# MGI-tech-bioinformatics/SuperPlus

Hardware: AMD Instinct MI355X
Metric: k-mers/s (DF createDict stage: trim + canonical k-mer count + solid filter + spectrum + adjacency) (higher is better)
Workload: dtype u64

## Files before the change

### superplus_amd/csrc/dfk.hip

```cpp
#include "../../include/dfk.h"
#include "dfk_kernels.h"
#include "dfk_arena.h"

#include <algorithm>
#include <chrono>
#include <cstdarg>
#include <cstdio>
#include <cstdlib>
#include <cstring>
#include <atomic>
#include <fcntl.h>
#include <functional>
#include <new>
#include <string>
#include <sys/mman.h>
#include <sys/stat.h>
#include <unistd.h>
#include <condition_variable>
#include <memory>
#include <mutex>
#include <thread>
#include <vector>

using namespace dfk;
// ... 152 lines not shown
        budget += kept_budget; kept_budget = 0; kept_n_reads = 0;
    }
};

namespace {

struct Timer {
    hipEvent_t a{}, b{}; hipStream_t s;
    explicit Timer(hipStream_t st) : s(st) { (void)hipEventCreate(&a); (void)hipEventCreate(&b); }
    ~Timer() { (void)hipEventDestroy(a); (void)hipEventDestroy(b); }
    void start() { (void)hipEventRecord(a, s); }
    float stop() { (void)hipEventRecord(b, s); (void)hipEventSynchronize(b); float ms = 0; (void)hipEventElapsedTime(&ms, a, b); return ms; }
};

uint32_t ceil_log2(uint64_t v) { uint32_t b = 0; while ((1ull << b) < v) ++b; return b; }

template <int K>
int stage_trim(dfk_ctx* c, const Inputs& in, uint64_t* n_inst)
{
    DevBuf ctr; int rc = c->alloc(ctr, 32, "trim counters"); if (rc) return rc;
    HIP_TRY(hipMemsetAsync(ctr.p, 0, 32, c->stream));
    rc = c->alloc(c->good_len, sizeof(uint32_t) * in.n_reads, "goodLens", Place::Low); if (rc) return rc;
    if (in.n_reads) {
        unsigned grid = (unsigned)std::min<uint64_t>((in.n_reads + 255) / 256, 8192);
        hipLaunchKernelGGL(HIP_KERNEL_NAME(k_trim<K>), dim3(grid), dim3(256), 0, c->stream,
                           in.pq, in.pq_off, in.pq_bytes, in.base_off, in.packed_bytes, in.read_len, in.n_reads, c->cfg.min_qual, (uint32_t*)c->good_len.p,
                           (unsigned long long*)ctr.p, (unsigned int*)((char*)ctr.p + 8),
                           (unsigned long long*)((char*)ctr.p + 16));
        HIP_TRY(hipGetLastError());
    }
    uint64_t h[3] = {0, 0, 0};
    HIP_TRY(hipMemcpyAsync(h, ctr.p, 24, hipMemcpyDeviceToHost, c->stream));
    HIP_TRY(hipStreamSynchronize(c->stream));
    c->release(ctr);
    if ((uint32_t)h[1]) return fail(DFK_E_INPUT, "malformed input: an offset table is not monotone or runs past its array, a PQVec stream is broken, or its length differs from read_len");
    if (h[2] == 0) return fail(DFK_E_NOGOOD, "Looks like your input data have almost no good bases.");
    *n_inst = h[0];
    return 0;
}

int device_scan(dfk_ctx* c, const uint64_t* in, uint64_t* out, uint64_t n)
{
    constexpr uint64_t PER = (uint64_t)SCAN_THREADS * SCAN_ITEMS;
    if (n == 0) return 0;
    const uint64_t nblk = (n + PER - 1) / PER;
    if (nblk == 1) {
        hipLaunchKernelGGL(k_scan_blocks, dim3(1), dim3(SCAN_THREADS), 0, c->stream, in, out, n, (uint64_t*)nullptr);
// ... 125 lines not shown
    J->count_due = false;
    return 0;
}

template <int K>
int scan_keys_piece(dfk_ctx* c, const Inputs& in, BucketTable* T, ScanJob* J, uint64_t r0, uint64_t r1)
{
    static const unsigned scan_blocks = getenv("DFK_SCAN_BLOCKS") ? (unsigned)atoi(getenv("DFK_SCAN_BLOCKS")) : 0;
    const unsigned cus = (unsigned)c->prop.multiProcessorCount;
    const unsigned grid = (unsigned)std::min<uint64_t>((r1 - r0 + PART_THREADS - 1) / PART_THREADS, (uint64_t)(scan_blocks ? scan_blocks : 128u) * cus);
    const uint64_t n_subs = (uint64_t)J->n_cls * J->n_sub;
    const bool two = J->n_slices > 1;
    const uint32_t sl = two ? (uint32_t)(J->n_pieces & 1) : 0;
    hipStream_t ks = two ? c->stream2 : c->stream;
    auto* cnt = (unsigned long long*)J->sub.p;
    auto* off = cnt + n_subs;
    auto* cur = off + n_subs + 1;
    ScanKeys sk = J->sk;
    sk.keys = (uint32_t*)J->keys.p + (uint64_t)sl * sk.cap * J->n_cls;
    sk.fill = (unsigned long long*)J->fill.p + (uint64_t)sl * J->n_cls;
    if (two && J->n_pieces >= 2) HIP_TRY(hipStreamWaitEvent(c->stream, J->ev_part[sl], 0));
    HIP_TRY(hipMemsetAsync(sk.fill, 0, J->n_cls * 8, c->stream));
    const size_t lds = SCAN_RUN_LDS + SCAN_STAGE_LDS;
    hipLaunchKernelGGL(HIP_KERNEL_NAME(k_scan_count<K, 16, true>), dim3(grid), dim3(PART_THREADS), lds, c->stream,
                       in.packed, in.packed_bytes, in.base_off, (const uint32_t*)c->good_len.p, r0, r1, J->pp,
                       (unsigned long long*)T->acc.p, (unsigned long long*)nullptr, (unsigned long long*)J->d_n.p, J->ovf_cap,
                       (uint32_t*)J->ovf_tmp.p, (uint4*)T->summ.p, (uint32_t*)T->classes.p, sk);
    HIP_TRY(hipGetLastError());
    if (two) {
        HIP_TRY(hipEventRecord(J->ev_scan, c->stream));
        if (J->count_due) { int rc = scan_keys_count(c, T, J); if (rc) return rc; }
        HIP_TRY(hipStreamWaitEvent(ks, J->ev_scan, 0));
        if (J->n_pieces >= 1) HIP_TRY(hipStreamWaitEvent(ks, J->ev_count, 0));
    }
    HIP_TRY(hipMemsetAsync(cnt, 0, n_subs * 8, ks));
    const dim3 per_class(std::max(1u, 16u * cus / J->n_cls), J->n_cls);
    const uint32_t sh = 6 + J->sb;
    hipLaunchKernelGGL(k_keys_subcount, per_class, dim3(256), J->n_sub * 4, ks,
                       (const uint32_t*)sk.keys, (const unsigned long long*)sk.fill, sk.cap, sh, J->n_sub, cnt);
    HIP_TRY(hipGetLastError());
    hipLaunchKernelGGL(k_keys_offsets, dim3(1), dim3(1024), 0, ks, (const unsigned long long*)cnt, (uint32_t)n_subs, off, cur);
    HIP_TRY(hipGetLastError());
    hipLaunchKernelGGL(k_keys_partition, per_class, dim3(256), J->n_sub * 12, ks,
                       (const uint32_t*)sk.keys, (const unsigned long long*)sk.fill, sk.cap, sh, J->n_sub, cur, (uint32_t*)J->keys2.p);
    HIP_TRY(hipGetLastError());
    if (two) HIP_TRY(hipEventRecord(J->ev_part[sl], ks));
    ++J->n_pieces; J->count_due = true;
// ... 18 lines not shown
int scan_range(dfk_ctx* c, const Inputs& in, BucketTable* T, ScanJob* J, uint64_t r0, uint64_t r1)
{
    if (r1 <= r0) return 0;
    const PartParams& pp = J->pp;
    const bool by_class = J->by_class;
    unsigned grid = (unsigned)((r1 - r0 + PART_THREADS - 1) / PART_THREADS);
    static const unsigned scan_blocks = getenv("DFK_SCAN_BLOCKS") ? (unsigned)atoi(getenv("DFK_SCAN_BLOCKS")) : 0;
    if (by_class) grid = std::min<unsigned>(grid, (scan_blocks ? scan_blocks : 128u) * (unsigned)c->prop.multiProcessorCount);
    else if (scan_blocks) grid = std::min<unsigned>(grid, scan_blocks * (unsigned)c->prop.multiProcessorCount);
    const size_t lds_a = (sizeof(uint32_t) + 1) * pp.W * PART_THREADS + sizeof(uint32_t) * PART_RING * PART_THREADS + (by_class ? J->n_bins * 4 : 0);
    hipEvent_t e0, e1;
    HIP_TRY(hipEventCreate(&e0)); HIP_TRY(hipEventCreate(&e1));
    J->ev.emplace_back(e0, e1);
    HIP_TRY(hipEventRecord(e0, c->stream));
    if (J->keyed) {
        uint64_t p0 = r0;
        for (uint64_t m : scan_piece_sizes(J, r1 - r0, r1 == in.n_reads)) {
            int rc = scan_keys_piece<K>(c, in, T, J, p0, p0 + m); if (rc) return rc;
            p0 += m;
        }
        if (r1 == in.n_reads && J->count_due) { int rc = scan_keys_count(c, T, J); if (rc) return rc; }
    } else if (scan_takes_ranges<K>(c)) {
        const size_t lds_r = SCAN_RUN_LDS + (by_class ? J->n_bins * 4 : 0);
        hipLaunchKernelGGL(HIP_KERNEL_NAME(k_scan_count<K, 16, false>), dim3(grid), dim3(PART_THREADS), lds_r, c->stream,
                           in.packed, in.packed_bytes, in.base_off, (const uint32_t*)c->good_len.p, r0, r1, pp,
                           (unsigned long long*)T->acc.p, (unsigned long long*)T->class_hist.p, (unsigned long long*)J->d_n.p, J->ovf_cap,
                           (uint32_t*)J->ovf_tmp.p, (uint4*)T->summ.p, (uint32_t*)T->classes.p, ScanKeys{});
    } else {
        if (r0 != 0 || r1 != in.n_reads) return fail(DFK_E_STATE, "the general scan takes every read at once");
        hipLaunchKernelGGL(HIP_KERNEL_NAME(k_partition<K, false>), dim3(grid), dim3(PART_THREADS), lds_a, c->stream,
                           in.packed, in.packed_bytes, in.base_off, (const uint32_t*)c->good_len.p, in.bc,
                           (int64_t)c->cfg.ign_bc_below, in.n_reads, pp, (unsigned long long*)T->acc.p, (unsigned long long*)T->class_hist.p,
                           (unsigned long long*)J->d_n.p, J->ovf_cap, (uint4*)J->ovf_tmp.p, (uint4*)T->summ.p,
                           (const uint32_t*)nullptr, (uint64_t)0, (const uint64_t*)nullptr, (uint32_t*)T->classes.p);
    }
    HIP_TRY(hipGetLastError());
    HIP_TRY(hipEventRecord(e1, c->stream));
    return 0;
}

template <int K>
int scan_end(dfk_ctx* c, const Inputs& in, uint64_t n_inst, BucketTable* T, ScanJob* J)
{
    int rc = 0;
    T->n_ovf = 0;
    if (J->count_due) { rc = scan_keys_count(c, T, J); if (rc) return rc; }
    c->release(J->keys); c->release(J->keys2); c->release(J->fill); c->release(J->sub);
// ... 81 lines not shown
    c->release(rec); c->release(inst); c->release(flags); c->release(idx);
    return 0;
}

void release_pass(dfk_ctx* c, Partition* P)
{ c->release(P->records); c->release(P->base); c->release(P->ipre); c->release(P->items); }

template <int K> uint64_t item_budget(const dfk_ctx* c)
{
    constexpr uint64_t S = 1ull << CountCfg<K>::LOG2S;
    if (c->cfg.inst_per_item) return c->cfg.inst_per_item;
    if (c->distinct_per_inst <= 0.0) return 3 * S / 2;
    const double b = 0.367 * (double)S / c->distinct_per_inst;
    return (uint64_t)std::min(std::max(b, 0.5 * (double)S), 3.0 * (double)S);
}

struct ScatterJob { Partition P; DevBuf cur, d_bad; hipStream_t st = nullptr; hipEvent_t e0 = nullptr, e1 = nullptr; uint32_t lo = 0, n = 0; };

template <int K>
int scatter_launch(dfk_ctx* c, const Inputs& in, const BucketTable& T, uint32_t log2_world, int64_t read_id0, ScatterJob* J)
{
    const PartParams pp = part_params<K>(c, T.log2_nb, log2_world, read_id0, J->lo, J->n);
    HIP_TRY(hipEventRecord(J->e0, J->st));
    if (in.n_reads)
        hipLaunchKernelGGL(HIP_KERNEL_NAME(k_scatter_runs<K>), dim3((unsigned)((in.n_reads + 256ull * sweep_reads<K>() - 1) / (256ull * sweep_reads<K>()))),
                           dim3(256), 0, J->st,
                           in.packed, in.packed_bytes, in.base_off, (const uint32_t*)c->good_len.p, in.bc,
                           (int64_t)c->cfg.ign_bc_below, in.n_reads, pp, (const uint4*)T.summ.p, (const uint32_t*)T.classes.p,
                           (unsigned long long*)J->cur.p, J->P.n_records, (uint4*)J->P.records.p);
    HIP_TRY(hipGetLastError());
    HIP_TRY(hipEventRecord(J->e1, J->st));
    return 0;
}

template <int K>
int scatter_begin(dfk_ctx* c, const Inputs& in, const BucketTable& T, uint32_t log2_world, int64_t read_id0,
                  uint32_t sub_lo, uint32_t sub_n, ScatterJob* J, bool launch_now = true)
{
    Partition* P = &J->P;
    J->st = c->stream; J->lo = sub_lo; J->n = sub_n;
    const PartParams pp = part_params<K>(c, T.log2_nb, log2_world, read_id0, sub_lo, sub_n);
    const uint64_t budget = item_budget<K>(c);
    int rc = pass_tables(c, T.acc, T.log2_nb - log2_world, 1u << log2_world, sub_lo, sub_n, budget, P); if (rc) return rc;
    const uint64_t nb = P->nb;
    rc = c->alloc(J->cur, nb * 8, "bucket cursors"); if (rc) return rc;
    rc = c->alloc(P->records, P->n_records * 32, "super-k-mer records"); if (rc) return rc;
    rc = c->alloc(J->d_bad, 16, "scatter check"); if (rc) return rc;
    HIP_TRY(hipMemcpyAsync(J->cur.p, P->base.p, nb * 8, hipMemcpyDeviceToDevice, c->stream));
// ... 24 lines not shown
                               (unsigned long long*)J->cur.p, P->n_records, (uint4*)P->records.p, (uint4*)nullptr,
                               (const uint32_t*)T.ovf_list.p, T.n_ovf, (const uint64_t*)nullptr, (uint32_t*)nullptr);
        HIP_TRY(hipGetLastError());
        hipLaunchKernelGGL(k_check_cursors, dim3((unsigned)std::min<uint64_t>((P->nb + 255) / 256, 4096)), dim3(256), 0, c->stream, (const unsigned long long*)J->cur.p,
                           (const uint64_t*)P->base.p, P->nb, (unsigned int*)J->d_bad.p);
        HIP_TRY(hipGetLastError());
        c->st.ms_part_scatter += t.stop();
    }
    unsigned int bad = 0;
    HIP_TRY(hipMemcpy(&bad, J->d_bad.p, 4, hipMemcpyDeviceToHost));
    c->release(J->d_bad); c->release(J->cur);
    if (bad) return fail(DFK_E_HIP, "scatter: %u buckets did not receive the records counted for them (run summaries and bucket counters disagree)", bad);
    TRACE("scatter of buckets [%u, %u) done (%llu records, %llu items)", J->lo, J->lo + J->n,
          (unsigned long long)J->P.n_records, (unsigned long long)J->P.n_items);
    return 0;
}

constexpr int E_SPLIT_NO_ROOM = -101;
constexpr int E_SEGMENT_FULL = -100;

struct CountRun {
    CountGlobals* g = nullptr; uint4* seg = nullptr; unsigned long long* hist = nullptr;
    CountParams cp{}; unsigned grid = 0;
    DevBuf big; uint64_t big_cap = 0;
    DevBuf d_hist, d_g;
    DevBuf d_snap;
    DevBuf d_part;
    DevBuf d_wg;
    uint64_t solid_seen = 0, inst_seen = 0;
    uint64_t boundary_seen = 0;
    uint64_t splits_seen = 0;
};

int count_run_begin(dfk_ctx* c, CountRun* R)
{
    int rc = c->alloc(R->d_hist, (uint64_t)HIST_GLOBAL_BINS * 8, "spectrum bins", Place::Low); if (rc) return rc;
    rc = c->alloc(R->d_g, sizeof(CountGlobals), "count globals", Place::Low); if (rc) return rc;
    HIP_TRY(hipMemsetAsync(R->d_hist.p, 0, (uint64_t)HIST_GLOBAL_BINS * 8, c->stream));
    HIP_TRY(hipMemsetAsync(R->d_g.p, 0, sizeof(CountGlobals), c->stream));
    R->g = (CountGlobals*)R->d_g.p; R->hist = (unsigned long long*)R->d_hist.p;
    return c->alloc(R->d_snap, (uint64_t)HIST_GLOBAL_BINS * 8 + 256, "spectrum snapshot", Place::Low);
}

int count_snapshot(dfk_ctx* c, CountRun* R, bool restore)
{
    char* snap = (char*)R->d_snap.p;
// ... 27 lines not shown
#endif
    DevBuf d_max; int rc = c->alloc(d_max, 16, "max bin"); if (rc) return rc;
    HIP_TRY(hipMemsetAsync(d_max.p, 0, 16, c->stream));
    hipLaunchKernelGGL(k_hist_max, dim3(1024), dim3(256), 0, c->stream, (const unsigned long long*)R->d_hist.p, HIST_GLOBAL_BINS,
                       (unsigned int*)d_max.p);
    uint32_t nb = 0;
    HIP_TRY(hipMemcpyAsync(&nb, d_max.p, 4, hipMemcpyDeviceToHost, c->stream));
    HIP_TRY(hipStreamSynchronize(c->stream));
    c->hist.assign(nb, 0);
    if (nb) HIP_TRY(hipMemcpy(c->hist.data(), R->d_hist.p, 8ull * nb, hipMemcpyDeviceToHost));
    TRACE("spectrum read back: %u bins, %llu solid", nb, (unsigned long long)c->n_solid);
    c->release(d_max); c->release(R->d_hist); c->release(R->d_g); c->release(R->d_snap);
    return 0;
}

template <int K> unsigned count_grid(const dfk_ctx* c, int nbc = 1)
{
    constexpr int LOG2S = CountCfg<K>::LOG2S, NW = CountCfg<K>::NWAVES;
    const size_t lds = count_lds_bytes<K, LOG2S, NW, 1>() + (size_t)(nbc > 1 ? nbc - 1 : 0) * sizeof(uint32_t) * (1u << LOG2S);
    const unsigned per_cu = (unsigned)std::max<size_t>(1, (size_t)(160 * 1024) / lds);
    return (unsigned)c->prop.multiProcessorCount * per_cu;
}

int launch_boundary_list(dfk_ctx* c)
{
    if (c->pending_blist < 0) return 0;
    const dfk_ctx::Part& part = c->parts[(size_t)c->pending_blist];
    c->pending_blist = -1;
    unsigned long long* ctl = (unsigned long long*)((char*)part.buf.p + part.blist);
    HIP_TRY(hipMemsetAsync(ctl, 0, 16, c->stream2));
    hipLaunchKernelGGL(k_boundary_list, dim3((unsigned)std::min<uint64_t>((part.n + 2047) / 2048, 4096)), dim3(256), 0, c->stream2,
                       (const uint4*)part.buf.p, part.n, (uint32_t*)(ctl + 2), part.n_blist, ctl);
    HIP_TRY(hipGetLastError());
    return 0;
}

template <int K, int NBC>
int launch_count(dfk_ctx* c, const Partition& P, const ItemRange* d_items, uint64_t n_items, const CountRun& R,
                 std::vector<ItemRange>* overflowed, float* kernel_ms, const uint32_t* d_sub = nullptr, bool single_kmer_records = false)
{
    constexpr int LOG2S = CountCfg<K>::LOG2S, NW = CountCfg<K>::NWAVES;
    if (n_items == 0) return 0;
    if (n_items >= (1ull << 32)) return fail(DFK_E_ARG, "too many work items in one pass");
    DevBuf d_ovf;
    int rc = c->alloc(d_ovf, n_items * sizeof(ItemRange), "overflow list"); if (rc) return rc;
    HIP_TRY(hipMemsetAsync(&R.g->next_item, 0, 8, c->stream));
    HIP_TRY(hipMemsetAsync(&R.g->n_wg_idle, 0, 4, c->stream));
    CountParams cp = R.cp; cp.n_items = (uint32_t)n_items; cp.single = single_kmer_records ? 1u : 0u;
    const size_t lds = count_lds_bytes<K, LOG2S, NW, NBC>();
    auto kern = d_sub ? k_count<K, LOG2S, NW, NBC, true> : k_count<K, LOG2S, NW, NBC, false>;
    HIP_TRY(hipFuncSetAttribute(reinterpret_cast<const void*>(kern), hipFuncAttributeMaxDynamicSharedMemorySize, (int)lds));
    TRACE("k_count: %llu items, grid %u, lds %zu, seg_cap %llu", (unsigned long long)n_items, R.grid, lds, (unsigned long long)R.cp.seg_cap);
    Timer tk(c->stream);
    tk.start();
    hipLaunchKernelGGL(kern, dim3(R.grid), dim3(NW * 64), lds, c->stream,
                       (const uint4*)P.records.p, d_items, (const uint64_t*)P.base.p, cp, R.g, R.seg, (WgOut*)R.d_wg.p, R.hist,
                       (ItemRange*)d_ovf.p, d_sub, c->d_resident);
    HIP_TRY(hipGetLastError());
    c->resident_target += R.grid;
    if (c->after_count_launch || c->pending_blist >= 0) {
        hipLaunchKernelGGL(k_gate, dim3(1), dim3(64), 0, c->stream2, (const unsigned int*)c->d_resident, c->resident_target, 200000ull, c->d_resident + 1);
    }
    if (c->after_count_launch) { std::function<int()> f; f.swap(c->after_count_launch); rc = f(); if (rc) return rc; }
    rc = launch_boundary_list(c); if (rc) return rc;
    *kernel_ms += tk.stop();
    CountGlobals g{};
    HIP_TRY(hipMemcpyAsync(&g, R.g, sizeof g, hipMemcpyDeviceToHost, c->stream));
    HIP_TRY(hipStreamSynchronize(c->stream));
    c->last_wg_idle = g.n_wg_idle;
    if (g.n_overflow) {
        const size_t at = overflowed->size();
        overflowed->resize(at + g.n_overflow);
        HIP_TRY(hipMemcpy(overflowed->data() + at, d_ovf.p, sizeof(ItemRange) * g.n_overflow, hipMemcpyDeviceToHost));
    }
    c->release(d_ovf);
    return 0;
}

template <int K, int NBC>
int launch_count_big(dfk_ctx* c, const Partition& P, const std::vector<ItemRange>& singles, CountRun& R)
{
    constexpr int KW = KTraits<K>::KW, NW = 8;
    const uint32_t n = (uint32_t)singles.size();
    std::vector<uint32_t> idx(2 * n);
    for (uint32_t i = 0; i < n; ++i) { idx[2 * i] = singles[i].b0; idx[2 * i + 1] = singles[i].b1; }
    DevBuf d_idx, d_val;
    int rc = c->alloc(d_idx, 8ull * n, "gather index"); if (rc) return rc;
    rc = c->alloc(d_val, 16ull * n, "gather values"); if (rc) return rc;
    HIP_TRY(hipMemcpyAsync(d_idx.p, idx.data(), 8ull * n, hipMemcpyHostToDevice, c->stream));
    hipLaunchKernelGGL(k_gather_u64, dim3((2 * n + 255) / 256), dim3(256), 0, c->stream, (const uint64_t*)P.ipre.p,
                       (const uint32_t*)d_idx.p, 2 * n, (uint64_t*)d_val.p);
    HIP_TRY(hipGetLastError());
    std::vector<uint64_t> val(2 * n);
    HIP_TRY(hipMemcpyAsync(val.data(), d_val.p, 16ull * n, hipMemcpyDeviceToHost, c->stream));
    HIP_TRY(hipStreamSynchronize(c->stream));
    c->release(d_idx); c->release(d_val);
    std::vector<BigItem> items; uint64_t words = 0, tot_inst = 0;
    std::vector<uint64_t> chunk_pre(n + 1, 0), slot_pre(n + 1, 0), rec(2 * n);
    {
// ... 175 lines not shown
        DevBuf d_next; rc = c->alloc(d_next, next.size() * sizeof(ItemRange), "split items"); if (rc) return undo(rc);
        HIP_TRY(hipMemcpyAsync(d_next.p, next.data(), next.size() * sizeof(ItemRange), hipMemcpyHostToDevice, c->stream));
        rc = launch_count<K, NBC>(c, P2, (const ItemRange*)d_next.p, next.size(), R, &overflowed, &ignored, nullptr, true);
        if (rc) return undo(rc);
    }
    TRACE("fallback: %u buckets (%llu instances) split into %llu sub-buckets, %llu items; %zu sub-buckets to HBM tables", n, (unsigned long long)tot,
          (unsigned long long)ns, (unsigned long long)P2.n_items, singles.size());
    if (!singles.empty()) { rc = launch_count_big<K, NBC>(c, P2, singles, R); if (rc) return undo(rc); }
    HIP_TRY(hipStreamSynchronize(c->stream));
    c->release_since(mark, &R.big);
    return 0;
}

int barcode_words(const dfk_ctx* c, bool have_bc)
{ return !have_bc ? 0 : (int)std::max<uint32_t>(1, std::min<uint32_t>(c->cfg.min_bc, DFK_MAX_MIN_BC) - (c->cfg.min_bc > 1 ? 1 : 0)); }

template <int K> constexpr uint64_t out_chunk() { return 2ull << CountCfg<K>::LOG2S; }

template <int K>
int count_prepare(dfk_ctx* c, const Partition& P, CountRun& R, int nbc)
{
    const unsigned attempt = c->seg_attempt;
    R.grid = (unsigned)std::max<uint64_t>(1, std::min<uint64_t>(P.n_items, count_grid<K>(c, nbc)));
    uint64_t res = part_entries(P.n_inst, c->cfg.min_freq, R.inst_seen, R.solid_seen);
    res = (res << attempt) + (uint64_t)R.grid * out_chunk<K>();
    const uint64_t room = c->budget > c->held ? (c->budget - c->held) : 0;
    if (res * 32 > room) res = room / 32;
    int rc = c->alloc(R.d_wg, sizeof(WgOut) * R.grid, "workgroup output state"); if (rc) return rc;
    std::vector<WgOut> init(R.grid, WgOut{~0ull, (unsigned int)out_chunk<K>(), 0u});
    HIP_TRY(hipMemcpy(R.d_wg.p, init.data(), sizeof(WgOut) * R.grid, hipMemcpyHostToDevice));
    HIP_TRY(hipMemsetAsync(&R.g->big_cursor, 0, 8, c->stream));
    HIP_TRY(hipMemsetAsync(&R.g->part_cursor, 0, 8, c->stream));
    R.cp = CountParams{c->cfg.min_freq, c->cfg.min_bc, 0, 0, res, c->cfg.min_freq > 1 ? 1u : 0u,
                       (c->cfg.flags & DFK_F_KEEP_PRE_ADJ) ? 1u : 0u};
    R.big_cap = 0;
    rc = c->alloc(R.d_part, std::max<uint64_t>(1, res) * 32, "solid k-mer entries", Place::Low); if (rc) return rc;
    R.seg = (uint4*)R.d_part.p;
    return 0;
}

template <int K, int NBC>
int count_run(dfk_ctx* c, const Partition& P, CountRun& R)
{
    int rc = 0;
    Timer t(c->stream);
    std::vector<ItemRange> overflowed;
// ... 360 lines not shown
            if (r != DFK_E_NOMEM || forced || n <= 16 || ++retries > 12) return r;
            c->plan_derate *= 0.7;
            TRACE("out of HBM (%s): planning smaller passes", g_err.c_str());
        }
    };
    rc = start_alone(cur, 0); if (rc) return rc;
    while (cur.valid) {
        const uint32_t lo = cur.sj.lo, n = cur.sj.n, nlo = lo + n;
        rc = scatter_end<K>(c, in, T, 0, 0, &cur.sj); if (rc) return rc;
        const dfk_stats st0 = c->st;
        rc = count_snapshot(c, &R, false); if (rc) return rc;
        { Arena::Current in_blk(c->arena, cur.blk); rc = count_prepare<K>(c, cur.sj.P, R, barcode_words(c, in.bc != nullptr)); }
        nxt.valid = false;
        if (!rc && overlap && nlo < sub_nb) {
            const Partition& P = cur.sj.P;
            (void)P;
            const RunningPass rp{cur.blk.block.bytes, cur.sj.P.n_inst, n, c->arena.offset_of(cur.blk.block)};
            const uint32_t n2 = forced ? std::min(per_forced, sub_nb - nlo) : plan_range(plan_inputs(c, T, R, sub_nb, nlo, overlap), c->arena.free_blocks(), &rp);
            if (n2) {
                const int r2 = start(nxt, nlo, n2, true);
                if (r2 && r2 != DFK_E_NOMEM) return r2;
            }
        }
        if (!rc) {
            switch (barcode_words(c, in.bc != nullptr)) {
            case 0: rc = count_run<K, 0>(c, cur.sj.P, R); break;
            case 1: rc = count_run<K, 1>(c, cur.sj.P, R); break;
            case 2: rc = count_run<K, 2>(c, cur.sj.P, R); break;
            case 3: rc = count_run<K, 3>(c, cur.sj.P, R); break;
            case 4: rc = count_run<K, 4>(c, cur.sj.P, R); break;
            case 5: rc = count_run<K, 5>(c, cur.sj.P, R); break;
            case 6: rc = count_run<K, 6>(c, cur.sj.P, R); break;
            default: rc = count_run<K, 7>(c, cur.sj.P, R); break;
            }
        }
        if (c->after_count_launch) {
            std::function<int()> f; f.swap(c->after_count_launch);
            if (!rc) { const int r3 = f(); if (r3) return r3; } else nxt.valid = false;
        }
        if (rc == DFK_E_NOMEM || rc == E_SEGMENT_FULL) {
            HIP_TRY(hipStreamSynchronize(c->stream)); HIP_TRY(hipStreamSynchronize(c->stream2));
            c->release_since(cur.mark);
            R.d_wg = R.big = R.d_part = DevBuf{};
            drop_events(cur); drop_events(nxt); nxt.valid = false;
            int rc2 = count_snapshot(c, &R, true); if (rc2) return rc2;
            const float ms_scatter = c->st.ms_part_scatter, ms_count = c->st.ms_count, ms_fb = c->st.ms_fallback;
// ... 689 lines not shown
```

### superplus_amd/csrc/dfk_kernels.h

```cpp
#pragma once
#include <type_traits>
#include "dfk_device.h"

namespace dfk {

template <int K>
__global__ void __launch_bounds__(256)
k_trim(const uint8_t* __restrict__ pq, const uint64_t* __restrict__ pq_off, uint64_t pq_nbytes,
       const uint64_t* __restrict__ base_off, uint64_t packed_bytes, const uint32_t* __restrict__ read_len,
       uint64_t n_reads, uint32_t min_qual, uint32_t* __restrict__ good_len,
       unsigned long long* __restrict__ n_inst, unsigned int* __restrict__ bad,
       unsigned long long* __restrict__ sum_good)
{
    unsigned long long mine = 0, good = 0;
    bool any_bad = false;
    for (uint64_t r = (uint64_t)blockIdx.x * blockDim.x + threadIdx.x; r < n_reads; r += (uint64_t)gridDim.x * blockDim.x) {
        uint32_t gl = 0;
        uint64_t p = pq_off[r], end = pq_off[r + 1];
        uint32_t idx = 0, run = 0;
        const uint64_t b0 = base_off[r], b1 = base_off[r + 1];
        bool ok = p <= end && end <= pq_nbytes && b0 <= b1 && b1 <= packed_bytes && b1 - b0 >= ((uint64_t)read_len[r] + 3) / 4;
        if (!ok) end = p;
        while (p < end) {
            uint32_t nQs = pq[p];
            if (!nQs) break;
            if (p + 3 > end) { ok = false; break; }
            uint32_t hdr = pq[p + 1] | ((uint32_t)pq[p + 2] << 8);
            uint32_t nBits = hdr & 7u, minQ = (hdr >> 3) & 63u;
            uint64_t blk = ((uint64_t)nQs * nBits + 24) >> 3;
            if (p + blk > end) { ok = false; break; }
            if (nBits == 0) {
                if (minQ >= min_qual) { run += nQs; if (run >= (uint32_t)K) gl = idx + nQs; }
                else run = 0;
                idx += nQs;
            } else {
                uint64_t bit = 8 * (p + 1) + 9;
                const uint32_t fmask = (1u << nBits) - 1u;
                for (uint32_t left = nQs; left;) {
                    const uint64_t by = bit >> 3;
                    const uint32_t sh = (uint32_t)(bit & 7);
                    uint64_t w = 0;
                    if (by + 8 <= pq_nbytes) __builtin_memcpy(&w, pq + by, 8);
                    else for (uint32_t k = 0; k < 8 && by + k < pq_nbytes; ++k) w |= (uint64_t)pq[by + k] << (8 * k);
                    w >>= sh;
                    const uint32_t n = min(left, (64u - sh) / nBits);
                    for (uint32_t i = 0; i < n; ++i, w >>= nBits) {
                        const uint32_t q = minQ + ((uint32_t)w & fmask);
                        if (q < min_qual) run = 0;
                        else if (++run >= (uint32_t)K) gl = idx + 1;
                        ++idx;
                    }
                    bit += (uint64_t)n * nBits; left -= n;
                }
            }
            p += blk;
        }
        uint32_t rl = read_len[r];
        if (!ok || idx != rl) { any_bad = true; gl = 0; }
        if (gl > rl) gl = rl;
        good_len[r] = gl;
        good += gl;
        if (gl >= (uint32_t)K + 1) mine += gl - K + 1;
    }
    __shared__ unsigned long long sh[2][4];
    __shared__ unsigned int sh_bad;
    if (threadIdx.x == 0) sh_bad = 0;
    __syncthreads();
#pragma unroll
    for (int d = 32; d > 0; d >>= 1) { mine += __shfl_down(mine, d, 64); good += __shfl_down(good, d, 64); }
    if ((threadIdx.x & 63) == 0) { sh[0][threadIdx.x >> 6] = mine; sh[1][threadIdx.x >> 6] = good; }
    if (any_bad) atomicOr(&sh_bad, 1u);
    __syncthreads();
    if (threadIdx.x == 0) {
        unsigned long long a0 = sh[0][0] + sh[0][1] + sh[0][2] + sh[0][3], a1 = sh[1][0] + sh[1][1] + sh[1][2] + sh[1][3];
        if (a0) atomicAdd(n_inst, a0);
        if (a1) atomicAdd(sum_good, a1);
        if (sh_bad) atomicOr(bad, 1u);
    }
}

struct PartParams {
    uint32_t M;
    uint32_t W;
    uint32_t log2_nb;
    uint32_t log2_world;
// ... 6 lines not shown
constexpr uint32_t SWEEP_CLASSES = 32;
__host__ __device__ inline uint32_t sweep_class_of(uint32_t local_bucket, uint32_t log2_local)
{ return log2_local > 5 ? local_bucket >> (log2_local - 5) : local_bucket; }
__host__ __device__ inline uint32_t sweep_class_mask(uint32_t sub_lo, uint32_t sub_n, uint32_t log2_local)
{
    if (sub_n == 0) return 0u;
    const uint32_t a = sweep_class_of(sub_lo, log2_local), b = sweep_class_of(sub_lo + sub_n - 1, log2_local);
    const uint32_t upto_b = b >= 31 ? 0xFFFFFFFFu : ((1u << (b + 1)) - 1u);
    return upto_b & ~((1u << a) - 1u);
}

constexpr int PART_THREADS = 128;
constexpr int PART_RING = 2;
constexpr int SUMMARY_RUNS = 10;
constexpr uint32_t SUMMARY_OVERFLOW = 15;

__device__ __forceinline__ uint32_t pass_local(uint32_t bucket, const PartParams& pp)
{
    const uint32_t ls = pp.log2_nb - pp.log2_world;
    const uint32_t d = (bucket & ((1u << ls) - 1u)) - pp.sub_lo;
    return d < pp.sub_n ? (bucket >> ls) * pp.sub_n + d : 0xFFFFFFFFu;
}

__device__ __forceinline__ uint32_t bucket_of(uint32_t minhash, const PartParams& pp)
{
    const uint32_t b = (minhash * 0x9E3779B1u) >> (32 - pp.log2_nb);
    return ((b & ((1u << pp.log2_world) - 1u)) << (pp.log2_nb - pp.log2_world)) | (b >> pp.log2_world);
}
constexpr int PART_QCAP = 8;

template <int K>
__device__ __forceinline__ void emit_record(const uint32_t* __restrict__ words, uint64_t n_words, uint64_t bit0,
                                            uint32_t s0, uint32_t nk, uint32_t bucket, uint32_t gl, int32_t tag,
                                            uint64_t dst_index, uint4* __restrict__ records)
{
    const bool hp = s0 > 0;
    const bool hs = s0 + nk + (uint32_t)K <= gl;
    uint64_t bo = bit0 + 2ull * (hp ? s0 - 1 : 0);
    uint64_t wi = bo >> 5; uint32_t sh = (uint32_t)bo & 31u;
    uint32_t w[7];
#pragma unroll
    for (int i = 0; i < 7; ++i) w[i] = (wi + i < n_words) ? words[wi + i] : 0u;
    uint32_t o[6];
#pragma unroll
    for (int i = 0; i < 6; ++i) o[i] = alignbit(w[i + 1], w[i], sh);
    if (!hp) {
#pragma unroll
        for (int i = 5; i > 0; --i) o[i] = (o[i] << 2) | (o[i - 1] >> 30);
        o[0] <<= 2;
// ... 213 lines not shown
                                 bucket_acc, bucket_cur, n_out, records, summaries, read_list, n_list, slice_base, read_classes);
    if (lh) {
        __syncthreads();
        for (uint32_t i = threadIdx.x; i < n_bins; i += PART_THREADS) if (lh[i]) atomicAdd(&class_hist[i], (unsigned long long)lh[i]);
    }
}

template <int I, int N, class F>
__device__ __forceinline__ void static_for(F&& f)
{
    if constexpr (I < N) { f(std::integral_constant<int, I>{}); static_for<I + 1, N>(f); }
}

struct ScanKeys {
    uint32_t* keys;
    unsigned long long* fill;
    uint64_t cap;
    uint32_t ib;
};
constexpr int SCAN_STAGE = 1536;
constexpr uint32_t KEY_SUB_BITS = 14;
constexpr uint32_t KEY_TILE = 4096;

template <int K, int M, bool KEYS>
__global__ void __launch_bounds__(PART_THREADS)
k_scan_count(const uint8_t* __restrict__ packed, uint64_t packed_bytes, const uint64_t* __restrict__ base_off,
             const uint32_t* __restrict__ good_len, uint64_t r_first, uint64_t n_reads , PartParams pp,
             unsigned long long* __restrict__ bucket_acc, unsigned long long* __restrict__ class_hist,
             unsigned long long* __restrict__ ovf_count, uint64_t ovf_cap, uint32_t* __restrict__ ovf_list,
             uint4* __restrict__ summaries, uint32_t* __restrict__ read_classes, ScanKeys sk)
{
    constexpr int W = K - M + 1;
    constexpr uint32_t mmask = M == 16 ? 0xFFFFFFFFu : ((1u << (2 * M)) - 1u);
    constexpr uint32_t rsh = 2 * (M - 1);
    constexpr int RUNS = SUMMARY_RUNS;
    static_assert(KTraits<K>::NK_MAX < 64, "nk takes the key's six low bits");
    extern __shared__ uint32_t smem[];
    uint32_t* runb = smem;
    uint16_t* runf = reinterpret_cast<uint16_t*>(runb + RUNS * PART_THREADS);
    uint32_t* const after_runs = reinterpret_cast<uint32_t*>(runf + RUNS * PART_THREADS);
    uint32_t* lh = nullptr;
    const uint32_t n_bins = 2u * (PART_CLASSES << pp.log2_world);
    if (class_hist) {
        lh = after_runs;
        for (uint32_t i = threadIdx.x; i < n_bins; i += PART_THREADS) lh[i] = 0;
        __syncthreads();
    }
// ... 79 lines not shown
                uint32_t a[NA];
                {
                    const uint32_t sh = (uint32_t)nbit & 31u;
#pragma unroll
                    for (int i = 0; i < NA; ++i) a[i] = alignbit(i + 1 < NW ? nw[i + 1] : 0u, nw[i], sh);
                }
                nbit += 2 * W;
                load(nbit, nw);
                static_for<0, W>([&](auto bi_c) {
                    constexpr int bi = decltype(bi_c)::value;
                    if (t0 + (uint32_t)bi < n_mmers) {
                        const uint32_t b = (a[(2 * bi) >> 5] >> ((2 * bi) & 31)) & 3u;
                        f = ((f << 2) | b) & mmask;
                        rc = (rc >> 2) | ((3u - b) << rsh);
                        const uint32_t h = mmer_hash(f < rc ? f : rc);
                        const bool newmin = bi == 0 || h < P;
                        P = newmin ? h : P;
                        Pi = newmin ? (uint32_t)bi : Pi;
                        const bool first = t0 == 0;
                        if (!first || bi == W - 1) {
                            uint32_t mv = P;
                            bool older = false;
                            if constexpr (bi != W - 1) { older = arr[bi + 1] < mv; mv = older ? arr[bi + 1] : mv; }
                            const uint32_t bucket = bucket_of(mv, pp);
                            const bool open = first || bucket != cur_b || cur_nk == (uint32_t)KTraits<K>::NK_MAX;
                            if (open && !first) close_run();
                            const uint32_t rel = (bi != W - 1 && older) ? sidx_get(bi + 1 < W ? bi + 1 : 0) - (uint32_t)bi - 1u : (uint32_t)(W - 1 - bi) + Pi;
                            cur_rel = open ? rel : cur_rel;
                            cur_nk = open ? 1u : cur_nk + 1u;
                            cur_b = open ? bucket : cur_b;
                        }
                        arr[bi] = h;
                        if (bi == W - 1) {
                            uint32_t run = h, ri = W - 1;
                            sidx_set(W - 1, W - 1);
                            static_for<0, W - 1>([&](auto j_c) {
                                constexpr int i = W - 2 - decltype(j_c)::value;
                                const bool lt = arr[i] < run; run = lt ? arr[i] : run; arr[i] = run; ri = lt ? (uint32_t)i : ri; sidx_set(i, ri);
                            });
                        }
                    }
                });
            }
            close_run();
        }
        const uint32_t mine = min(qn, (uint32_t)RUNS);
        for (uint32_t i = 0; KEYS ? __syncthreads_or(i < mine) != 0 : __ballot(i < mine) != 0ull; ++i) {
// ... 146 lines not shown
        key_tile_each(t0, t1, v, [&](uint32_t key) { const uint32_t s = key >> sh2; out[base[s] + atomicAdd(&lh[s], 1u)] = key; });
        __syncthreads();
    }
}

__global__ void __launch_bounds__(1024)
k_keys_count(const uint32_t* __restrict__ part, const unsigned long long* __restrict__ off, uint32_t sb, unsigned long long* __restrict__ bucket_acc)
{
    __shared__ unsigned long long t[1u << KEY_SUB_BITS];
    const uint32_t s = blockIdx.x, nt = 1u << sb, m = nt - 1u;
    for (uint32_t i = threadIdx.x; i < nt; i += blockDim.x) t[i] = 0;
    __syncthreads();
    const uint64_t a = off[s], b = off[s + 1];
    for (uint64_t i = a + threadIdx.x; i < b; i += blockDim.x) {
        const uint32_t key = part[i];
        atomicAdd(&t[(key >> 6) & m], (1ull << 32) | (key & 63u));
    }
    __syncthreads();
    unsigned long long* dst = bucket_acc + ((uint64_t)s << sb);
    for (uint32_t i = threadIdx.x; i < nt; i += blockDim.x) if (t[i]) atomicAdd(&dst[i], t[i]);
}

constexpr int SLICE_READS = 16;
template <int K, bool EMIT, typename F>
__device__ __forceinline__ void for_each_run_in_pass(uint64_t r, const uint8_t* __restrict__ packed, uint64_t packed_bytes,
                                                     const uint64_t* __restrict__ base_off, const PartParams& pp,
                                                     const uint4* __restrict__ summaries, F&& f)
{
    const uint4 sm = summaries[r];
    const uint32_t n = sm.x & 15u;
    if (n == 0 || n == SUMMARY_OVERFLOW) return;
    const uint32_t* words = reinterpret_cast<const uint32_t*>(packed);
    const uint64_t n_words = (packed_bytes + 3) >> 2;
    const uint64_t bit0 = base_off[r] * 8;
    const uint32_t M = pp.M;
    const uint32_t mmask = M == 16 ? 0xFFFFFFFFu : ((1u << (2 * M)) - 1u);
    const uint64_t lo = (uint64_t)sm.x | ((uint64_t)sm.y << 32), hi = (uint64_t)sm.z | ((uint64_t)sm.w << 32);
    uint32_t s0 = 0;
#pragma unroll
    for (int i = 0; i < SUMMARY_RUNS; ++i) {
        if ((uint32_t)i < n) {
            constexpr int B0 = 8;
            const int b = B0 + 12 * i;
            const uint32_t fld = (uint32_t)(b + 12 <= 64 ? lo >> b : b >= 64 ? hi >> (b - 64) : (lo >> b) | (hi << (64 - b))) & 0xFFFu;
            const uint32_t nk = fld & 63u, rel = fld >> 6;
            const uint64_t bo = bit0 + 2ull * (s0 + rel);
            const uint64_t wi = bo >> 5;
            const uint32_t w0 = words[wi], w1 = wi + 1 < n_words ? words[wi + 1] : 0u;
            const uint32_t x = alignbit(w1, w0, (uint32_t)bo & 31u) & mmask;
            uint32_t y = __brev(x);
            y = ((y >> 1) & 0x55555555u) | ((y & 0x55555555u) << 1);
            const uint32_t fw = y >> (32 - 2 * M), rcv = ~x & mmask;
            const uint32_t bucket = bucket_of(mmer_hash(fw < rcv ? fw : rcv), pp);
            const uint32_t lb = pass_local(bucket, pp);
            if (lb != 0xFFFFFFFFu) f(s0, nk, lb, bucket >> (pp.log2_nb - pp.log2_world), bit0, (uint32_t)i + 1 == n);
            s0 += nk;
        }
    }
}

template <int K>
__global__ void __launch_bounds__(256)
k_scatter_slices(const uint8_t* __restrict__ packed, uint64_t packed_bytes, const uint64_t* __restrict__ base_off,
                 const uint32_t* __restrict__ good_len, const int32_t* __restrict__ bc, int64_t ign_bc_below,
                 uint64_t n_reads, PartParams pp, const uint4* __restrict__ summaries, const uint32_t* __restrict__ read_classes,
                 const uint64_t* __restrict__ slice_base,
                 unsigned long long* __restrict__ slice_fill,
                 uint4* __restrict__ records)
{
    __shared__ uint32_t cnt[256];
    __shared__ unsigned long long at[256];
    __shared__ uint16_t list[256 * SLICE_READS];
    __shared__ uint32_t n_list;
    const uint32_t world = 1u << pp.log2_world;
    const int lane = threadIdx.x & 63;
    const uint64_t r_block = (uint64_t)blockIdx.x * 256 * SLICE_READS;
// ... 22 lines not shown
        at[threadIdx.x] = slice_base[threadIdx.x] + (m ? atomicAdd(&slice_fill[threadIdx.x], (unsigned long long)m) : 0ull);
        cnt[threadIdx.x] = 0;
    }
    __syncthreads();
    const uint32_t* words = reinterpret_cast<const uint32_t*>(packed);
    const uint64_t n_words = (packed_bytes + 3) >> 2;
    (void)good_len;
    for (uint32_t i = threadIdx.x; i < n; i += 256) {
        const uint64_t r = r_block + list[i];
        int32_t tag = -1;
        if (bc && (int64_t)r + pp.read_id0 >= ign_bc_below) tag = bc[r];
        for_each_run_in_pass<K, true>(r, packed, packed_bytes, base_off, pp, summaries,
            [&](uint32_t s0, uint32_t nk, uint32_t lb, uint32_t owner, uint64_t bit0, bool last) {
                const uint64_t dst = at[owner] + atomicAdd(&cnt[owner], 1u);
                if (dst < slice_base[owner + 1]) emit_record<K>(words, n_words, bit0, s0, nk, lb, last ? 0u : 0xFFFFFFFFu, tag, dst, records);
            });
    }
}

#ifndef DFK_SWEEP_READS
#define DFK_SWEEP_READS 8
#endif
template <int K> constexpr int sweep_reads() { return KTraits<K>::KW == 4 ? 2 : DFK_SWEEP_READS; }
template <int K>
__global__ void __launch_bounds__(256)
k_scatter_runs(const uint8_t* __restrict__ packed, uint64_t packed_bytes, const uint64_t* __restrict__ base_off,
               const uint32_t* __restrict__ good_len, const int32_t* __restrict__ bc, int64_t ign_bc_below,
               uint64_t n_reads, PartParams pp, const uint4* __restrict__ summaries, const uint32_t* __restrict__ read_classes,
               unsigned long long* __restrict__ bucket_cur, uint64_t n_out, uint4* __restrict__ records)
{
    constexpr int SWEEP_READS = sweep_reads<K>();
    __shared__ uint16_t list[256 * SWEEP_READS];
    __shared__ uint32_t n_list;
    (void)good_len;
    const int lane = threadIdx.x & 63;
    const uint64_t r_block = (uint64_t)blockIdx.x * 256 * SWEEP_READS;
    if (threadIdx.x == 0) n_list = 0;
    __syncthreads();
#pragma unroll
    for (int j = 0; j < SWEEP_READS; ++j) {
        const uint32_t rel = 256u * j + threadIdx.x;
        const uint64_t r = r_block + rel;
        const bool hit = r < n_reads && (read_classes[r] & pp.class_mask) != 0u;
        const unsigned long long mk = __ballot(hit);
        uint32_t at = 0;
        if (lane == 0 && mk) at = atomicAdd(&n_list, (uint32_t)__popcll(mk));
        at = __builtin_amdgcn_readfirstlane(at);
        if (hit) list[at + __popcll(mk & ((1ull << lane) - 1ull))] = (uint16_t)rel;
    }
    __syncthreads();
    const uint32_t n = n_list;
    const uint32_t* words = reinterpret_cast<const uint32_t*>(packed);
    const uint64_t n_words = (packed_bytes + 3) >> 2;
    for (uint32_t i = threadIdx.x; i < n; i += 256) {
        const uint64_t r = r_block + list[i];
        int32_t tag = -1;
        if (bc && (int64_t)r + pp.read_id0 >= ign_bc_below) tag = bc[r];
        for_each_run_in_pass<K, true>(r, packed, packed_bytes, base_off, pp, summaries,
            [&](uint32_t s0, uint32_t nk, uint32_t lb, uint32_t, uint64_t bit0, bool last) {
                const uint64_t dst = atomicAdd(&bucket_cur[lb], 1ull);
                if (dst < n_out) emit_record<K>(words, n_words, bit0, s0, nk, lb, last ? 0u : 0xFFFFFFFFu, tag, dst, records);
            });
    }
}



struct ItemRange { uint32_t b0, b1; };

struct CountParams {
    uint32_t min_freq, min_bc;
    uint32_t n_items;
    uint32_t single;
    uint64_t seg_cap;
    uint32_t do_adj;
    uint32_t keep_pre;
};

struct CountGlobals {
    unsigned long long n_distinct;
    unsigned long long big_cursor;
// ... 1466 lines not shown
```

Before: 64.75 billion.

## Batch trim reads per thread, specialize single-device bucketing, add wider count shape

The trim kernel now has each thread prefetch offsets and the first quality header for two reads before walking them. It also handles a leading constant-quality block without the byte loop, and the grid is sized from occupancy. Scan and scatter kernels gain a SOLO template path that skips the world-interleave arithmetic in bucket_of when log2_world is zero. The count kernel can also launch with 12 waves per block when the LDS fits two blocks per CU and there is at most one barcode word, which raises parallelism per block at the cost of more template instantiations.

```diff
diff --git a/superplus_amd/csrc/dfk.hip b/superplus_amd/csrc/dfk.hip
--- a/superplus_amd/csrc/dfk.hip
+++ b/superplus_amd/csrc/dfk.hip
@@ -198,7 +198,10 @@
     HIP_TRY(hipMemsetAsync(ctr.p, 0, 32, c->stream));
     rc = c->alloc(c->good_len, sizeof(uint32_t) * in.n_reads, "goodLens", Place::Low); if (rc) return rc;
     if (in.n_reads) {
-        unsigned grid = (unsigned)std::min<uint64_t>((in.n_reads + 255) / 256, 8192);
+        const uint64_t per_block = 256ull * TRIM_READS;
+        int per_cu = 0;
+        HIP_TRY(hipOccupancyMaxActiveBlocksPerMultiprocessor(&per_cu, reinterpret_cast<const void*>(&k_trim<K>), 256, 0));
+        unsigned grid = (unsigned)std::min<uint64_t>((in.n_reads + per_block - 1) / per_block, (uint64_t)std::max(1, per_cu) * (uint64_t)c->prop.multiProcessorCount);
         hipLaunchKernelGGL(HIP_KERNEL_NAME(k_trim<K>), dim3(grid), dim3(256), 0, c->stream,
                            in.pq, in.pq_off, in.pq_bytes, in.base_off, in.packed_bytes, in.read_len, in.n_reads, c->cfg.min_qual, (uint32_t*)c->good_len.p,
                            (unsigned long long*)ctr.p, (unsigned int*)((char*)ctr.p + 8),
@@ -370,7 +373,8 @@
     if (two && J->n_pieces >= 2) HIP_TRY(hipStreamWaitEvent(c->stream, J->ev_part[sl], 0));
     HIP_TRY(hipMemsetAsync(sk.fill, 0, J->n_cls * 8, c->stream));
     const size_t lds = SCAN_RUN_LDS + SCAN_STAGE_LDS;
-    hipLaunchKernelGGL(HIP_KERNEL_NAME(k_scan_count<K, 16, true>), dim3(grid), dim3(PART_THREADS), lds, c->stream,
+    auto kern = J->pp.log2_world == 0 ? k_scan_count<K, 16, true, true> : k_scan_count<K, 16, true, false>;
+    hipLaunchKernelGGL(kern, dim3(grid), dim3(PART_THREADS), lds, c->stream,
                        in.packed, in.packed_bytes, in.base_off, (const uint32_t*)c->good_len.p, r0, r1, J->pp,
                        (unsigned long long*)T->acc.p, (unsigned long long*)nullptr, (unsigned long long*)J->d_n.p, J->ovf_cap,
                        (uint32_t*)J->ovf_tmp.p, (uint4*)T->summ.p, (uint32_t*)T->classes.p, sk);
@@ -435,7 +439,8 @@
         if (r1 == in.n_reads && J->count_due) { int rc = scan_keys_count(c, T, J); if (rc) return rc; }
     } else if (scan_takes_ranges<K>(c)) {
         const size_t lds_r = SCAN_RUN_LDS + (by_class ? J->n_bins * 4 : 0);
-        hipLaunchKernelGGL(HIP_KERNEL_NAME(k_scan_count<K, 16, false>), dim3(grid), dim3(PART_THREADS), lds_r, c->stream,
+        auto kern = (pp.log2_world == 0 && !by_class) ? k_scan_count<K, 16, false, true> : k_scan_count<K, 16, false, false>;
+        hipLaunchKernelGGL(kern, dim3(grid), dim3(PART_THREADS), lds_r, c->stream,
                            in.packed, in.packed_bytes, in.base_off, (const uint32_t*)c->good_len.p, r0, r1, pp,
                            (unsigned long long*)T->acc.p, (unsigned long long*)T->class_hist.p, (unsigned long long*)J->d_n.p, J->ovf_cap,
                            (uint32_t*)J->ovf_tmp.p, (uint4*)T->summ.p, (uint32_t*)T->classes.p, ScanKeys{});
@@ -563,8 +568,9 @@
 {
     const PartParams pp = part_params<K>(c, T.log2_nb, log2_world, read_id0, J->lo, J->n);
     HIP_TRY(hipEventRecord(J->e0, J->st));
+    auto kern = log2_world == 0 ? k_scatter_runs<K, true> : k_scatter_runs<K, false>;
     if (in.n_reads)
-        hipLaunchKernelGGL(HIP_KERNEL_NAME(k_scatter_runs<K>), dim3((unsigned)((in.n_reads + 256ull * sweep_reads<K>() - 1) / (256ull * sweep_reads<K>()))),
+        hipLaunchKernelGGL(kern, dim3((unsigned)((in.n_reads + 256ull * sweep_reads<K>() - 1) / (256ull * sweep_reads<K>()))),
                            dim3(256), 0, J->st,
                            in.packed, in.packed_bytes, in.base_off, (const uint32_t*)c->good_len.p, in.bc,
                            (int64_t)c->cfg.ign_bc_below, in.n_reads, pp, (const uint4*)T.summ.p, (const uint32_t*)T.classes.p,
@@ -635,6 +641,7 @@
 struct CountRun {
     CountGlobals* g = nullptr; uint4* seg = nullptr; unsigned long long* hist = nullptr;
     CountParams cp{}; unsigned grid = 0;
+    int nwaves = 0;
     DevBuf big; uint64_t big_cap = 0;
     DevBuf d_hist, d_g;
     DevBuf d_snap;
@@ -708,6 +715,19 @@
     return (unsigned)c->prop.multiProcessorCount * per_cu;
 }
 
+constexpr int LONE_WAVES = 12;
+template <int K, int NBC> constexpr bool lone_shape_fits()
+{
+    constexpr int LOG2S = CountCfg<K>::LOG2S, NW = CountCfg<K>::NWAVES;
+    return NW < LONE_WAVES && 2 * count_lds_bytes<K, LOG2S, LONE_WAVES, NBC>() <= (size_t)(160 * 1024)
+        && (size_t)(160 * 1024) / count_lds_bytes<K, LOG2S, NW, NBC>() == 2;
+}
+template <int K> void count_lone_shape(CountRun& R, int nbc)
+{
+    const char* e = getenv("DFK_LONE_WAVES");
+    if ((!e || atoi(e) == LONE_WAVES) && nbc <= 1 && lone_shape_fits<K, 1>()) R.nwaves = LONE_WAVES;
+}
+
 int launch_boundary_list(dfk_ctx* c)
 {
     if (c->pending_blist < 0) return 0;
@@ -721,11 +741,11 @@
     return 0;
 }
 
-template <int K, int NBC>
-int launch_count(dfk_ctx* c, const Partition& P, const ItemRange* d_items, uint64_t n_items, const CountRun& R,
-                 std::vector<ItemRange>* overflowed, float* kernel_ms, const uint32_t* d_sub = nullptr, bool single_kmer_records = false)
-{
-    constexpr int LOG2S = CountCfg<K>::LOG2S, NW = CountCfg<K>::NWAVES;
+template <int K, int NBC, int NW>
+int launch_count_shape(dfk_ctx* c, const Partition& P, const ItemRange* d_items, uint64_t n_items, const CountRun& R,
+                       std::vector<ItemRange>* overflowed, float* kernel_ms, const uint32_t* d_sub, bool single_kmer_records)
+{
+    constexpr int LOG2S = CountCfg<K>::LOG2S;
     if (n_items == 0) return 0;
     if (n_items >= (1ull << 32)) return fail(DFK_E_ARG, "too many work items in one pass");
     DevBuf d_ovf;
@@ -761,6 +781,15 @@
     }
     c->release(d_ovf);
     return 0;
+}
+
+template <int K, int NBC>
+int launch_count(dfk_ctx* c, const Partition& P, const ItemRange* d_items, uint64_t n_items, const CountRun& R,
+                 std::vector<ItemRange>* overflowed, float* kernel_ms, const uint32_t* d_sub = nullptr, bool single_kmer_records = false)
+{
+    if constexpr (lone_shape_fits<K, NBC>())
+        if (R.nwaves == LONE_WAVES) return launch_count_shape<K, NBC, LONE_WAVES>(c, P, d_items, n_items, R, overflowed, kernel_ms, d_sub, single_kmer_records);
+    return launch_count_shape<K, NBC, CountCfg<K>::NWAVES>(c, P, d_items, n_items, R, overflowed, kernel_ms, d_sub, single_kmer_records);
 }
 
 template <int K, int NBC>
@@ -982,6 +1011,7 @@
 {
     const unsigned attempt = c->seg_attempt;
     R.grid = (unsigned)std::max<uint64_t>(1, std::min<uint64_t>(P.n_items, count_grid<K>(c, nbc)));
+    R.nwaves = CountCfg<K>::NWAVES;
     uint64_t res = part_entries(P.n_inst, c->cfg.min_freq, R.inst_seen, R.solid_seen);
     res = (res << attempt) + (uint64_t)R.grid * out_chunk<K>();
     const uint64_t room = c->budget > c->held ? (c->budget - c->held) : 0;
@@ -1388,6 +1418,7 @@
                 if (r2 && r2 != DFK_E_NOMEM) return r2;
             }
         }
+        if (!rc && !nxt.valid) count_lone_shape<K>(R, barcode_words(c, in.bc != nullptr));
         if (!rc) {
             switch (barcode_words(c, in.bc != nullptr)) {
             case 0: rc = count_run<K, 0>(c, cur.sj.P, R); break;
diff --git a/superplus_amd/csrc/dfk_kernels.h b/superplus_amd/csrc/dfk_kernels.h
--- a/superplus_amd/csrc/dfk_kernels.h
+++ b/superplus_amd/csrc/dfk_kernels.h
@@ -4,6 +4,21 @@
 
 namespace dfk {
 
+constexpr int TRIM_READS = 2;
+__device__ __forceinline__ uint64_t pq_load8(const uint8_t* __restrict__ pq, uint64_t at, uint64_t nbytes)
+{
+    uint64_t w = 0;
+    if (at + 8 <= nbytes) __builtin_memcpy(&w, pq + at, 8);
+    else {
+#pragma unroll
+        for (uint32_t k = 0; k < 8; ++k) {
+            const uint64_t i = at + k;
+            const uint32_t b = pq[i < nbytes ? i : nbytes - 1];
+            w |= (uint64_t)(i < nbytes ? b : 0u) << (8 * k);
+        }
+    }
+    return w;
+}
 template <int K>
 __global__ void __launch_bounds__(256)
 k_trim(const uint8_t* __restrict__ pq, const uint64_t* __restrict__ pq_off, uint64_t pq_nbytes,
@@ -14,53 +29,80 @@
 {
     unsigned long long mine = 0, good = 0;
     bool any_bad = false;
-    for (uint64_t r = (uint64_t)blockIdx.x * blockDim.x + threadIdx.x; r < n_reads; r += (uint64_t)gridDim.x * blockDim.x) {
-        uint32_t gl = 0;
-        uint64_t p = pq_off[r], end = pq_off[r + 1];
-        uint32_t idx = 0, run = 0;
-        const uint64_t b0 = base_off[r], b1 = base_off[r + 1];
-        bool ok = p <= end && end <= pq_nbytes && b0 <= b1 && b1 <= packed_bytes && b1 - b0 >= ((uint64_t)read_len[r] + 3) / 4;
-        if (!ok) end = p;
-        while (p < end) {
-            uint32_t nQs = pq[p];
-            if (!nQs) break;
-            if (p + 3 > end) { ok = false; break; }
-            uint32_t hdr = pq[p + 1] | ((uint32_t)pq[p + 2] << 8);
-            uint32_t nBits = hdr & 7u, minQ = (hdr >> 3) & 63u;
-            uint64_t blk = ((uint64_t)nQs * nBits + 24) >> 3;
-            if (p + blk > end) { ok = false; break; }
-            if (nBits == 0) {
-                if (minQ >= min_qual) { run += nQs; if (run >= (uint32_t)K) gl = idx + nQs; }
-                else run = 0;
-                idx += nQs;
-            } else {
-                uint64_t bit = 8 * (p + 1) + 9;
-                const uint32_t fmask = (1u << nBits) - 1u;
-                for (uint32_t left = nQs; left;) {
-                    const uint64_t by = bit >> 3;
-                    const uint32_t sh = (uint32_t)(bit & 7);
-                    uint64_t w = 0;
-                    if (by + 8 <= pq_nbytes) __builtin_memcpy(&w, pq + by, 8);
-                    else for (uint32_t k = 0; k < 8 && by + k < pq_nbytes; ++k) w |= (uint64_t)pq[by + k] << (8 * k);
-                    w >>= sh;
-                    const uint32_t n = min(left, (64u - sh) / nBits);
-                    for (uint32_t i = 0; i < n; ++i, w >>= nBits) {
-                        const uint32_t q = minQ + ((uint32_t)w & fmask);
-                        if (q < min_qual) run = 0;
-                        else if (++run >= (uint32_t)K) gl = idx + 1;
-                        ++idx;
-                    }
-                    bit += (uint64_t)n * nBits; left -= n;
+    const uint64_t stride = (uint64_t)gridDim.x * blockDim.x;
+    for (uint64_t r0 = (uint64_t)blockIdx.x * blockDim.x + threadIdx.x; r0 < n_reads; r0 += TRIM_READS * stride) {
+        uint64_t p[TRIM_READS], end[TRIM_READS], b0[TRIM_READS], b1[TRIM_READS], w[TRIM_READS];
+        uint32_t rl[TRIM_READS];
+        bool live[TRIM_READS], ok[TRIM_READS];
+#pragma unroll
+        for (int u = 0; u < TRIM_READS; ++u) {
+            const uint64_t r = r0 + u * stride;
+            live[u] = r < n_reads;
+            p[u] = end[u] = b0[u] = b1[u] = 0; rl[u] = 0;
+            if (live[u]) { p[u] = pq_off[r]; end[u] = pq_off[r + 1]; b0[u] = base_off[r]; b1[u] = base_off[r + 1]; rl[u] = read_len[r]; }
+        }
+#pragma unroll
+        for (int u = 0; u < TRIM_READS; ++u) {
+            ok[u] = p[u] <= end[u] && end[u] <= pq_nbytes && b0[u] <= b1[u] && b1[u] <= packed_bytes && b1[u] - b0[u] >= ((uint64_t)rl[u] + 3) / 4;
+            if (!ok[u]) end[u] = p[u];
+            w[u] = p[u] < end[u] ? pq_load8(pq, p[u], pq_nbytes) : 0ull;
+        }
+#pragma unroll
+        for (int u = 0; u < TRIM_READS; ++u) {
+            if (!live[u]) continue;
+            const uint64_t r = r0 + u * stride;
+            uint32_t gl = 0, idx = 0, run = 0;
+            uint64_t pp = p[u];
+            const uint64_t e = end[u];
+            bool okk = ok[u];
+            bool walk = pp < e;
+            if (walk) {
+                const uint32_t nQs = (uint32_t)w[u] & 255u, hdr = (uint32_t)(w[u] >> 8) & 0xFFFFu;
+                if (!nQs) walk = false;
+                else if (pp + 3 <= e && (hdr & 7u) == 0) {
+                    if (((hdr >> 3) & 63u) >= min_qual) { run = nQs; if (run >= (uint32_t)K) gl = nQs; }
+                    idx = nQs;
+                    pp += 3;
+                    walk = pp < e && ((uint32_t)(w[u] >> 24) & 255u) != 0;
                 }
             }
-            p += blk;
-        }
-        uint32_t rl = read_len[r];
-        if (!ok || idx != rl) { any_bad = true; gl = 0; }
-        if (gl > rl) gl = rl;
-        good_len[r] = gl;
-        good += gl;
-        if (gl >= (uint32_t)K + 1) mine += gl - K + 1;
+            if (walk) while (pp < e) {
+                uint32_t nQs = pq[pp];
+                if (!nQs) break;
+                if (pp + 3 > e) { okk = false; break; }
+                uint32_t hdr = pq[pp + 1] | ((uint32_t)pq[pp + 2] << 8);
+                uint32_t nBits = hdr & 7u, minQ = (hdr >> 3) & 63u;
+                uint64_t blk = ((uint64_t)nQs * nBits + 24) >> 3;
+                if (pp + blk > e) { okk = false; break; }
+                if (nBits == 0) {
+                    if (minQ >= min_qual) { run += nQs; if (run >= (uint32_t)K) gl = idx + nQs; }
+                    else run = 0;
+                    idx += nQs;
+                } else {
+                    uint64_t bit = 8 * (pp + 1) + 9;
+                    const uint32_t fmask = (1u << nBits) - 1u;
+                    for (uint32_t left = nQs; left;) {
+                        const uint64_t by = bit >> 3;
+                        const uint32_t sh = (uint32_t)(bit & 7);
+                        uint64_t q8 = pq_load8(pq, by, pq_nbytes) >> sh;
+                        const uint32_t n = min(left, (64u - sh) / nBits);
+                        for (uint32_t i = 0; i < n; ++i, q8 >>= nBits) {
+                            const uint32_t q = minQ + ((uint32_t)q8 & fmask);
+                            if (q < min_qual) run = 0;
+                            else if (++run >= (uint32_t)K) gl = idx + 1;
+                            ++idx;
+                        }
+                        bit += (uint64_t)n * nBits; left -= n;
+                    }
+                }
+                pp += blk;
+            }
+            if (!okk || idx != rl[u]) { any_bad = true; gl = 0; }
+            if (gl > rl[u]) gl = rl[u];
+            good_len[r] = gl;
+            good += gl;
+            if (gl >= (uint32_t)K + 1) mine += gl - K + 1;
+        }
     }
     __shared__ unsigned long long sh[2][4];
     __shared__ unsigned int sh_bad;
@@ -113,9 +155,11 @@
     return d < pp.sub_n ? (bucket >> ls) * pp.sub_n + d : 0xFFFFFFFFu;
 }
 
+template <bool SOLO = false>
 __device__ __forceinline__ uint32_t bucket_of(uint32_t minhash, const PartParams& pp)
 {
     const uint32_t b = (minhash * 0x9E3779B1u) >> (32 - pp.log2_nb);
+    if constexpr (SOLO) return b;
     return ((b & ((1u << pp.log2_world) - 1u)) << (pp.log2_nb - pp.log2_world)) | (b >> pp.log2_world);
 }
 constexpr int PART_QCAP = 8;
@@ -375,7 +419,7 @@
 constexpr uint32_t KEY_SUB_BITS = 14;
 constexpr uint32_t KEY_TILE = 4096;
 
-template <int K, int M, bool KEYS>
+template <int K, int M, bool KEYS, bool SOLO = false>
 __global__ void __launch_bounds__(PART_THREADS)
 k_scan_count(const uint8_t* __restrict__ packed, uint64_t packed_bytes, const uint64_t* __restrict__ base_off,
              const uint32_t* __restrict__ good_len, uint64_t r_first, uint64_t n_reads , PartParams pp,
@@ -501,7 +545,7 @@
                             uint32_t mv = P;
                             bool older = false;
                             if constexpr (bi != W - 1) { older = arr[bi + 1] < mv; mv = older ? arr[bi + 1] : mv; }
-                            const uint32_t bucket = bucket_of(mv, pp);
+                            const uint32_t bucket = bucket_of<SOLO>(mv, pp);
                             const bool open = first || bucket != cur_b || cur_nk == (uint32_t)KTraits<K>::NK_MAX;
                             if (open && !first) close_run();
                             const uint32_t rel = (bi != W - 1 && older) ? sidx_get(bi + 1 < W ? bi + 1 : 0) - (uint32_t)bi - 1u : (uint32_t)(W - 1 - bi) + Pi;
@@ -694,7 +738,7 @@
 }
 
 constexpr int SLICE_READS = 16;
-template <int K, bool EMIT, typename F>
+template <int K, bool EMIT, bool SOLO = false, typename F>
 __device__ __forceinline__ void for_each_run_in_pass(uint64_t r, const uint8_t* __restrict__ packed, uint64_t packed_bytes,
                                                      const uint64_t* __restrict__ base_off, const PartParams& pp,
                                                      const uint4* __restrict__ summaries, F&& f)
@@ -723,7 +767,7 @@
             uint32_t y = __brev(x);
             y = ((y >> 1) & 0x55555555u) | ((y & 0x55555555u) << 1);
             const uint32_t fw = y >> (32 - 2 * M), rcv = ~x & mmask;
-            const uint32_t bucket = bucket_of(mmer_hash(fw < rcv ? fw : rcv), pp);
+            const uint32_t bucket = bucket_of<SOLO>(mmer_hash(fw < rcv ? fw : rcv), pp);
             const uint32_t lb = pass_local(bucket, pp);
             if (lb != 0xFFFFFFFFu) f(s0, nk, lb, bucket >> (pp.log2_nb - pp.log2_world), bit0, (uint32_t)i + 1 == n);
             s0 += nk;
@@ -792,7 +836,7 @@
 #define DFK_SWEEP_READS 8
 #endif
 template <int K> constexpr int sweep_reads() { return KTraits<K>::KW == 4 ? 2 : DFK_SWEEP_READS; }
-template <int K>
+template <int K, bool SOLO = false>
 __global__ void __launch_bounds__(256)
 k_scatter_runs(const uint8_t* __restrict__ packed, uint64_t packed_bytes, const uint64_t* __restrict__ base_off,
                const uint32_t* __restrict__ good_len, const int32_t* __restrict__ bc, int64_t ign_bc_below,
@@ -826,7 +870,7 @@
         const uint64_t r = r_block + list[i];
         int32_t tag = -1;
         if (bc && (int64_t)r + pp.read_id0 >= ign_bc_below) tag = bc[r];
-        for_each_run_in_pass<K, true>(r, packed, packed_bytes, base_off, pp, summaries,
+        for_each_run_in_pass<K, true, SOLO>(r, packed, packed_bytes, base_off, pp, summaries,
             [&](uint32_t s0, uint32_t nk, uint32_t lb, uint32_t, uint64_t bit0, bool last) {
                 const uint64_t dst = atomicAdd(&bucket_cur[lb], 1ull);
                 if (dst < n_out) emit_record<K>(words, n_words, bit0, s0, nk, lb, last ? 0u : 0xFFFFFFFFu, tag, dst, records);
```

Result: no change. 65.17 billion (median of 6 runs) (+0.6%).
